# JJanai/slowflow

Measured on AMD Instinct MI355X. Metric: Mpix*solver-iters/s at 1024x436 (whole coarse-to-fine path), higher is better.
Workload: dtype f32

## Files before the change

slowflow_amd/csrc/job.hip:

```cpp
#include <algorithm>
#include <cmath>
#include <cstring>
#include <memory>
#include <vector>

#include "sfa_internal.h"

#pragma clang fp contract(off)

namespace sfa {

enum { P_WX = 0, P_WY, P_UU, P_VV, P_DU, P_DV, P_ODU, P_ODV, P_SH, P_SV, P_A11, P_A12, P_A22, P_B1, P_B2, P_OCC, P_DPSIS, P_COUNT };
struct Level {
    int w = 0, h = 0, pitch = 0, lstride = 0, ref = 0, F = 0, nb = 0;
    bool fused = true;
    long pl = 0, es = 0;
    long off_masks = 0, off_warp = 0, off_stacks = 0, off_tmp = 0;
    float *base = nullptr;
    float *pbase = nullptr;
    float *plane(int i) const { return i < 2 ? pbase + (long)i * pl : base + (long)(i - 2) * pl; }
    float *mask(int s) const { return base + off_masks + (long)s * pl; }
    float *stack(int s, int toref) const { return base + off_stacks + ((long)s * 2 + toref) * 24 * pl; }
    float *warp(int s, int sp1) const { return base + off_warp + (long)(s + sp1) * 3 * pl; }
    float *frame(int f) const { return pbase + 2 * pl + (long)f * 3 * pl; }
    float *tmp() const { return base + off_tmp; }
    Geo geo() const { return Geo{w, h, pitch, pl, es, nb, WMask::first(nb), nullptr}; }
    Geo geo(const WMask &active) const { return Geo{w, h, pitch, pl, es, nb, active, nullptr}; }
    static long persistent_floats(int pitch, int h, int ref) { return (long)pitch * h * (2 + (2L * ref + 1) * 3); }
    static long transient_floats(int pitch, int h, int ref, bool fused) {
        return (long)pitch * h * ((P_COUNT - 2) + 2 * ref + (2L * ref + 1) * 3 + (fused ? 0 : 2L * ref * 2 * 24));
    }
    void layout(float *transient, float *persistent, int w_, int h_, int lstride_, int ref_, int nb_, long es_, bool fused_) {
        base = transient; pbase = persistent; w = w_; h = h_; pitch = dev_pitch(w_); lstride = lstride_; ref = ref_; F = 2 * ref_ + 1; nb = nb_; es = es_; fused = fused_;
        pl = (long)pitch * h;
        off_masks = (long)(P_COUNT - 2) * pl;
        off_warp = off_masks + 2L * ref * pl;
        off_stacks = off_warp + (2L * ref + 1) * 3 * pl;
        off_tmp = off_warp;
    }
};
struct ChannelWeights { const float *dev = nullptr; long pl = 0, es = 0; int pitch = 0, stride0 = 0; };

static const float *pair_image(const Level &L, int s, int sp1) { return (s + sp1 - L.ref == 0) ? L.frame(s + sp1) : L.warp(s, sp1); }

static bool get_derivatives(sfa_ctx *c, const Level &L, const sfa_params &p, const Geo &g, const bool need_toref[2 * SFA_MAX_REF], bool with_smoothness = false) {
    const int ref = L.ref;
    WarpJobs J;
    J.n = 0;
    for (int f = p.one_direction ? ref + 1 : 0; f <= 2 * ref; f++) {
        if (f == ref) continue;
        const int s = f < ref ? f : f - 1;
        J.job[J.n++] = WarpJob{L.frame(f) - L.base, L.warp(f < ref ? f : f - 1, f < ref ? 0 : 1) - L.base, L.mask(s) - L.base, f - ref};
    }
    const bool smoothed = with_smoothness && L.fused &&
                          launch_warp_smooth(c, g, J, L.base, L.plane(P_WX), L.plane(P_WY), p.smoothing, L.plane(P_SH), L.plane(P_SV), L.plane(P_DPSIS), p.alpha, pen(p.robust_reg));
    if (!smoothed) launch_warp_jobs(c, g, J, L.base, L.plane(P_WX), L.plane(P_WY));
    for (int s = p.one_direction ? ref : 0; s < 2 * ref; s++) {
        if (L.fused) continue;
        const float *w_s = pair_image(L, s, 0), *w_sp1 = pair_image(L, s, 1);
        launch_deriv_stack(c, g, L.stack(s, 0), w_s, w_sp1, L.es, L.es);
        if (need_toref[s]) {
            if (s < ref) launch_deriv_stack(c, g, L.stack(s, 1), w_s, L.frame(ref), L.es, L.es);
            else         launch_deriv_stack(c, g, L.stack(s, 1), L.frame(ref), w_sp1, L.es, L.es);
        }
    }
    return smoothed;
}

static int optimize_occlusions(sfa_ctx *c, const Level &L, const sfa_params &p, const Geo &g, DevMem &scratch) {
    const int ref = L.ref;
    const size_t n = (size_t)L.nb * L.pl;
    SFA_TRY(scratch.alloc(c, (2 + kCutWorkPlanes) * n * sizeof(float)));
    float *d0 = scratch.f(), *d1 = d0 + n, *work = d1 + n;
    OccArgs oa;
    memset(&oa, 0, sizeof oa);
    oa.nslots = 2 * ref; oa.hd = p.delta / 3.0f; oa.hg = p.gamma / 3.0f; oa.penalty = p.occlusion_penalty;
    oa.color = pen(p.robust_color); oa.grad = pen(p.robust_grad);
    for (int s = 0; s < 2 * ref; s++) {
        const float *i1 = pair_image(L, s, 0), *i2 = pair_image(L, s, 1);
        const float *r1 = s < ref ? i1 : L.frame(ref), *r2 = s < ref ? L.frame(ref) : i2;
        const int idx = std::max(ref - s - 1, s - ref);
        oa.slot[s] = OccSlot{i1 - L.base, i2 - L.base, r1 - L.base, r2 - L.base, L.off_masks + (long)s * L.pl, p.rho[idx], p.omega[idx], s >= ref ? 0 : 1};
    }
    launch_occ_costs(c, g, oa, L.base, d0, d1, L.pl);
    return run_grid_cut(c, g, L.plane(P_OCC), L.es, d0, d1, work, p.occlusion_alpha);
}


static Term data_term(const Level &L, const sfa_params &p, int slot, int is_ref, float weight, float s) {
    const float *i1 = pair_image(L, slot, 0), *i2 = pair_image(L, slot, 1);
    if (is_ref) { if (slot < L.ref) i2 = L.frame(L.ref); else i1 = L.frame(L.ref); }
    return Term{L.off_stacks + ((long)slot * 2 + is_ref) * 24 * L.pl, L.off_masks + (long)slot * L.pl, weight * (p.delta / 3.0f), weight * (p.gamma / 3.0f), s, is_ref,
                i1 - L.base, i2 - L.base, slot < L.ref};
}
static int data_terms(sfa_ctx *c, const Level &L, const sfa_params &p, const ChannelWeights &cw, AssembleArgs &aa, bool need_toref[2 * SFA_MAX_REF]) {
    const int ref = L.ref;
    memset(&aa, 0, sizeof aa);
    for (int s = 0; s < ref; s++) {
        const int a = ref - 1 - s;
        if (!p.one_direction) {
            if (p.rho[a] > 0) aa.t[aa.n++] = data_term(L, p, s, 0, p.rho[a], (float)(s - ref));
            if (p.omega[a] > 0) { aa.t[aa.n++] = data_term(L, p, s, 1, p.omega[a], (float)(s - ref)); need_toref[s] = true; }
        }
        if (p.rho[s] > 0) aa.t[aa.n++] = data_term(L, p, ref + s, 0, p.rho[s], (float)s);
        if (p.omega[s] > 0) { aa.t[aa.n++] = data_term(L, p, ref + s, 1, p.omega[s], (float)(s + 1)); need_toref[ref + s] = true; }
        aa.data_norm += p.rho[s] + p.omega[s];
    }
    for (int t = 0; t < aa.n; t++)
        if (aa.t[t].is_ref && aa.t[t].s == 0) return set_error(c, SFA_ERR_REF_FRAME, "Frame compared to reference frame is the reference frame itself!");
    aa.one_direction = p.one_direction; aa.dt_norm = p.dataterm_norm;
    aa.color = pen(p.robust_color); aa.grad = pen(p.robust_grad);
    aa.chw = cw.dev; aa.chw_pl = cw.pl; aa.chw_es = cw.es; aa.chw_pitch = cw.pitch; aa.chw_stride0 = cw.stride0; aa.lstride = L.lstride;
    aa.accumulate = 0; aa.do_laplacian = 1;
    return SFA_OK;
}

struct LevelPlan {
    bool verbose;
    bool red_black;
    bool direct;
    bool uv_alias;
    bool thres_in, thres_out;
    float *wx, *wy, *uu, *vv, *du, *dv, *odu, *odv, *sh, *sv, *a11, *a12, *a22, *b1, *b2, *occ, *dpsis, *UU, *VV;
    float *dfa, *dfb, *ifa, *ifb;
    LevelPlan(const sfa_ctx *c, const Level &L, const sfa_params &p) {
        verbose = c->verbose_changes;
        red_black = p.sor_order == 1;
        direct = L.fused && !red_black && !sw_given(Switches::NO_DIRECT_OPERANDS);
        uv_alias = direct && p.niter_inner == 1 && !sw_given(Switches::NO_UV_ALIAS) && !verbose;
        thres_in = p.thres_inner > 0; thres_out = p.thres_outer > 0;
        wx = L.plane(P_WX); wy = L.plane(P_WY); uu = L.plane(P_UU); vv = L.plane(P_VV); du = L.plane(P_DU); dv = L.plane(P_DV);
        odu = L.plane(P_ODU); odv = L.plane(P_ODV); sh = L.plane(P_SH); sv = L.plane(P_SV); a11 = L.plane(P_A11); a12 = L.plane(P_A12);
        a22 = L.plane(P_A22); b1 = L.plane(P_B1); b2 = L.plane(P_B2); occ = L.plane(P_OCC); dpsis = L.plane(P_DPSIS);
        UU = uv_alias ? wx : uu; VV = uv_alias ? wy : vv;
        dfa = thres_out && !sw_given(Switches::NO_EXACT_BREAK) ? a11 : nullptr; dfb = dfa ? a12 : nullptr;
        ifa = thres_in && !sw_given(Switches::NO_EXACT_BREAK) ? a11 : nullptr; ifb = ifa ? a12 : nullptr;
    }
};

struct OuterBreak {
    sfa_ctx *c; bool on;
    int known(int n, WMask &active) const {
        if (!on || n < kMaskLag) return SFA_OK;
        const int slot = (n - kMaskLag) % kMaskRing;
        SFA_HIP(c, hipEventSynchronize(c->ev_mask[slot]));
        for (int i = 0; i < kMaskWords; i++) active.w[i] = *(volatile unsigned long long *)&c->h_amask[slot].w[i];
        return SFA_OK;
    }
    int publish(int n) const {
        if (!on) return SFA_OK;
        const int slot = n % kMaskRing;
        SFA_HIP(c, hipMemcpyAsync(&c->h_amask[slot], c->d_amask, sizeof(WMask), hipMemcpyDeviceToHost, c->stream));
        SFA_HIP(c, hipEventRecord(c->ev_mask[slot], c->stream));
        return SFA_OK;
    }
};

static void print_changes(sfa_ctx *c, const Level &L, const char *what, int it, const WMask &who) {
    if (hipMemcpyAsync(c->h_red, c->d_red, 2 * L.nb * sizeof(double), hipMemcpyDeviceToHost, c->stream) != hipSuccess || hipStreamSynchronize(c->stream) != hipSuccess) return;
    const double n = (double)L.w * L.h;
    for (int b = 0; b < L.nb; b++)
        if (who.test(b)) {
            if (L.nb > 1) printf("[window %d] ", b);
            printf("%s %d\tavg change %g,%g\n", what, it, (double)(float)(c->h_red[2 * b] / n), (double)(float)(c->h_red[2 * b + 1] / n));
        }
    fflush(stdout);
}

static int assemble_and_solve(sfa_ctx *c, const Level &L, const sfa_params &p, const LevelPlan &P, AssembleArgs &aa, SorWorkspace &sorws, const Geo &gi, bool first_zero,
                       bool smoothed) {
    if (!first_zero) launch_copy_planes(c, gi, P.odu, P.du, 2, L.es, L.es);
    if (!smoothed) launch_smoothness(c, gi, p.smoothing, P.sh, P.sv, P.UU, P.VV, P.dpsis, p.alpha, pen(p.robust_reg));
    aa.op = SorOperandOut();
    aa.zero_duv = first_zero ? 1 : 0;
    if (P.direct) SFA_TRY(sor_operand_target(c, sorws, gi, p.niter_solver, &aa.op));
    if (L.fused) SFA_TRY(launch_assemble_images(c, gi, aa, L.base, P.a11, P.a12, P.a22, P.b1, P.b2, P.du, P.dv, P.UU, P.VV, P.sh, P.sv, P.occ));
    else launch_assemble(c, gi, aa, L.base, P.a11, P.a12, P.a22, P.b1, P.b2, P.du, P.dv, P.uu, P.vv, P.sh, P.sv);
    if (P.direct) return sor_run_prepared(c, sorws, gi, nullptr, nullptr, p.niter_solver, p.sor_omega);
    if (P.red_black) return sor_rb_run(c, gi, P.du, P.dv, P.a11, P.a12, P.a22, P.b1, P.b2, P.sh, P.sv, p.niter_solver, p.sor_omega);
    return sor_run(c, sorws, gi, P.du, P.dv, P.a11, P.a12, P.a22, P.b1, P.b2, P.sh, P.sv, p.niter_solver, p.sor_omega, false);
}

static bool update_flow(sfa_ctx *c, const sfa_params &p, const LevelPlan &P, const SorOperandOut &x, const Geo &gi, int inner, bool first_zero) {
    const bool last = inner + 1 == p.niter_inner;
    float *const ia = last ? nullptr : P.ifa, *const ib = last ? nullptr : P.ifb;
    if (P.direct && last && !P.verbose) {
        launch_update_outer_x(c, gi, P.uv_alias ? nullptr : P.uu, P.uv_alias ? nullptr : P.vv, P.wx, P.wy, x, c->d_red, P.dfa, P.dfb);
        return true;
    }
    if (P.direct)
        launch_update_inner_x(c, gi, P.uu, P.vv, P.wx, P.wy, x, first_zero ? nullptr : P.odu, first_zero ? nullptr : P.odv, last ? nullptr : P.du,
                              last ? nullptr : P.dv, c->d_red, ia, ib);
    else
        launch_update_inner(c, gi, P.uu, P.vv, P.wx, P.wy, P.du, P.dv, P.odu, P.odv, c->d_red, ia, ib);
    return false;
}

static int inner_break(sfa_ctx *c, const Level &L, const sfa_params &p, const LevelPlan &P, const Geo &gi, WMask &in_active) {
    const double npx = (double)L.h * L.w;
    SFA_HIP(c, hipMemcpyAsync(c->h_red, c->d_red, 2 * L.nb * sizeof(double), hipMemcpyDeviceToHost, c->stream));
    SFA_HIP(c, hipStreamSynchronize(c->stream));
    WMask close = WMask::none();
    for (int b = 0; b < L.nb; b++)
        if (in_active.test(b)) {
            const double ad = c->h_red[2 * b] / npx, dd = c->h_red[2 * b + 1] / npx, dm = (ad < dd) ? dd : ad;
            if (P.ifa && fabs(dm - (double)p.thres_inner) <= break_band(L.w, L.h) * (double)p.thres_inner) { close.set(b); continue; }
            if (std::max((float)ad, (float)dd) < p.thres_inner) in_active.clear(b);
        }
    if (!close.any()) return SFA_OK;
    float *const dx = c->d_last->exact;
    const float *const hx = reinterpret_cast<const LastBlock *>(c->h_red)->exact;
    launch_exact_norms(c, gi, P.ifa, P.ifb, close, dx);
    SFA_HIP(c, hipMemcpyAsync(const_cast<float *>(hx), dx, 2 * L.nb * sizeof(float), hipMemcpyDeviceToHost, c->stream));
    SFA_HIP(c, hipStreamSynchronize(c->stream));
    for (int b = 0; b < L.nb; b++)
        if (close.test(b) && std::max(hx[2 * b], hx[2 * b + 1]) < p.thres_inner) in_active.clear(b);
    return SFA_OK;
}

static int inner_iterations(sfa_ctx *c, const Level &L, const sfa_params &p, const LevelPlan &P, AssembleArgs &aa, SorWorkspace &sorws, const Geo &g, bool smoothed) {
    if (!P.direct) launch_zero_planes(c, g, P.du, 2);
    WMask in_active = g.active, outer_done = WMask::none();
    for (int inner = 0; inner < p.niter_inner; inner++) {
        Geo gi = g;
        gi.active = in_active;
        const bool first_zero = P.direct && inner == 0;
        SFA_TRY(assemble_and_solve(c, L, p, P, aa, sorws, gi, first_zero, smoothed && inner == 0));
        if (update_flow(c, p, P, aa.op, gi, inner, first_zero)) outer_done = in_active;
        if (P.verbose) print_changes(c, L, "\tinner it", inner, in_active);
// ... 457 lines not shown
```

slowflow_amd/csrc/kernels.hip:

```cpp
#include "sfa_device.h"
#include "sor_device.h"

#pragma clang fp contract(off)

namespace sfa {

__device__ __forceinline__ float psi_vec(const PenaltyDev &p, float xsq) {
    const float e2 = p.eps * p.eps;
    switch (p.id) {
    case 0: return 1.0f;
    case 2: return __fdiv_rn(1.0f, 2.0f * e2 + xsq);
    case 3: {
        float out = __fdiv_rn(1.0f, 2.0f * sqrt_rn(xsq + e2));
        if (sqrt_rn(xsq) > p.trunc) out = 0.0f;
        return out;
    }
    case 4: {
        float t = e2 + xsq;
        t = t * t;
        return __fdiv_rn(e2 + 2.0f * xsq, t);
    }
    default: return __fdiv_rn(1.0f, 2.0f * sqrt_rn(xsq + e2));
    }
}
__device__ __forceinline__ float psi_scalar(const PenaltyDev &p, float xsq) {
    const float e2f = p.eps * p.eps;
    const double e2d = (double)e2f;
    switch (p.id) {
    case 0: return 1.0f;
    case 2: return (float)(1.0 / (2.0 * e2d + (double)xsq));
    case 3:
        if (sqrt_rn(xsq) > p.trunc) return 0.0f;
        return __fdiv_rn(1.0f, 2.0f * sqrt_rn(xsq + e2f));
    case 4: {
        float t = (float)(e2d + (double)xsq);
        t = t * t;
        return (float)((e2d + (double)(2.0f * xsq)) / (double)t);
    }
    default: return (float)(1.0 / (2.0 * __dsqrt_rn((double)xsq + e2d)));
    }
}

__global__ void k_warp(float *__restrict__ dst3, float *__restrict__ mask, const float *__restrict__ src3, const float *__restrict__ wx,
                       const float *__restrict__ wy, Geo g, int factor, long src_es) {
    const int b = blockIdx.z;
    if (!elem_active(g, b)) return;
    const int x = blockIdx.x * BX + threadIdx.x, y = blockIdx.y * BY + threadIdx.y;
    if (x >= g.w || y >= g.h) return;
    dst3 += b * g.es; wx += b * g.es; wy += b * g.es; src3 += b * src_es;
    const size_t o = (size_t)y * g.pitch + x;
    if (factor == 0) {
        for (int k = 0; k < 3; k++) dst3[k * g.pl + o] = src3[k * g.pl + o];
        return;
    }
    const float xx = x + factor * wx[o];
    const float yy = y + factor * wy[o];
    const int xi = floor_to_int_x86(xx), yi = floor_to_int_x86(yy);
    const float dx = xx - xi, dy = yy - yi;
    if (mask) mask[b * g.es + o] = (xx >= 0 && xx <= g.w - 1 && yy >= 0 && yy <= g.h - 1) ? 1.0f : 0.0f;
    const int x1 = clampi(xi, 0, g.w - 1), x2 = clampi(xi + 1, 0, g.w - 1);
    const int y1 = clampi(yi, 0, g.h - 1), y2 = clampi(yi + 1, 0, g.h - 1);
    const float ax = 1.0f - dx, ay = 1.0f - dy;
    for (int k = 0; k < 3; k++) {
        const float *s = src3 + k * g.pl;
        dst3[k * g.pl + o] = s[(size_t)y1 * g.pitch + x1] * ax * ay + s[(size_t)y1 * g.pitch + x2] * dx * ay
                           + s[(size_t)y2 * g.pitch + x1] * ax * dy + s[(size_t)y2 * g.pitch + x2] * dx * dy;
    }
}
template <bool ALLJ>
__global__ void k_warp_jobs(WarpJobs J, float *__restrict__ base, const float *__restrict__ wx, const float *__restrict__ wy, Geo g) {
    const int b = ALLJ ? blockIdx.z : blockIdx.z / J.n, j0 = ALLJ ? 0 : blockIdx.z % J.n;
    if (!elem_active(g, b)) return;
    const int x = blockIdx.x * BX + threadIdx.x, y = blockIdx.y * BY + threadIdx.y;
    if (x >= g.w || y >= g.h) return;
    const long eb = b * g.es;
    const size_t o = (size_t)y * g.pitch + x;
    const float fx0 = wx[eb + o], fy0 = wy[eb + o];
    for (int j = j0; j <= (ALLJ ? J.n - 1 : j0); j++) {
        const int factor = J.job[j].factor;
        const float *src3 = base + eb + J.job[j].src_off;
        float *dst3 = base + eb + J.job[j].dst_off;
        const float xx = x + factor * fx0;
        const float yy = y + factor * fy0;
        const int xi = floor_to_int_x86(xx), yi = floor_to_int_x86(yy);
        const float dx = xx - xi, dy = yy - yi;
        if (J.job[j].mask_off >= 0) base[eb + J.job[j].mask_off + o] = (xx >= 0 && xx <= g.w - 1 && yy >= 0 && yy <= g.h - 1) ? 1.0f : 0.0f;
        const int x1 = clampi(xi, 0, g.w - 1), x2 = clampi(xi + 1, 0, g.w - 1);
        const int y1 = clampi(yi, 0, g.h - 1), y2 = clampi(yi + 1, 0, g.h - 1);
        const float ax = 1.0f - dx, ay = 1.0f - dy;
        float out[3];
#pragma unroll
        for (int k = 0; k < 3; k++) {
            const float *s = src3 + k * g.pl;
            out[k] = s[(size_t)y1 * g.pitch + x1] * ax * ay + s[(size_t)y1 * g.pitch + x2] * dx * ay
                   + s[(size_t)y2 * g.pitch + x1] * ax * dy + s[(size_t)y2 * g.pitch + x2] * dx * dy;
// ... 1226 lines not shown
        for (int ch = 0; ch < 3; ch++) {
            const TileAcc X{sX[ch], x0, y0 + 2}, Y{sY[ch], x0, y0 + 2}, Z{sZ[ch], x0, y0};
            p.ixy[ch] = d5y(X, xc_, y, g.h);
            p.iyy[ch] = d5y(Y, xc_, y, g.h);
            p.iyz[ch] = d5y(Z, xc_, y, g.h);
            p.ix[ch] = sX[ch][c]; p.iy[ch] = sY[ch][c]; p.iz[ch] = sZ[ch][cz];
            p.ixx[ch] = d5x_in(sX[ch], c);
            p.ixz[ch] = d5x_in(sZ[ch], cz);
        }
    }
    return p;
}
template <class K>
__device__ __forceinline__ void asm_epilogue_pixel(const AssembleArgs &a, const Geo &g, Acc &A, float u, float v, int x0, int y0, int tx, int yl, int x, int y) {
    const float *const lds = asm_lds<K>();
    const int gy0 = y0 + DT_H - 1;
    const TileAcc U{lds, x0, gy0}, V{lds + K::GR * DT_W, x0, gy0}, Hh{lds + 2 * K::GR * DT_W, x0, gy0}, Wv{lds + 3 * K::GR * DT_W, x0, gy0};
    if (a.do_laplacian) {
        A.b1 = laplacian_gather(A.b1, U, Hh, Wv, x, y, g.w, g.h);
        A.b2 = laplacian_gather(A.b2, V, Hh, Wv, x, y, g.w, g.h);
    }
    if (!a.op.sa) return;
    const float hp = Hh(x, y);
    const float hl = x > 0 ? Hh(x - 1, y) : 0.0f;
    const float vp = Wv(x, y);
    const float vt = y > 0 ? Wv(x, y - 1) : 0.0f;
    const PointBlock q = sor_point_block(hl, hp, vt, vp, y, g.h, A.a11, A.a12, A.a22);
    const OperandTile<K> T;
    T.A[yl][tx] = make_float4(q.i11, q.i12, q.i22, vt);
    T.B[yl][tx] = make_float4(A.b1, A.b2, hp, y < g.h - 1 ? vp : 0.0f);
    T.X[yl][tx] = make_float2(u, v);
}
template <class K>
__device__ __forceinline__ void asm_store_operand_tile(const SorOperandOut &op, const Geo &g, int b, int c0, int r0) {
    const OperandTile<K> T;
    for (int item = threadIdx.x; item < (DT_X + K::TY - 1) * K::TY; item += K::NT) {
        const int dl = item / K::TY, rl = item % K::TY, cl = dl - rl;
        if (cl < 0 || cl >= DT_X) continue;
        const int r = r0 + rl, c = c0 + cl;
        if (r >= g.h || c >= g.w) continue;
        const size_t e = diag_entry(b, op.ent, op.RP, op.G, c, r);
        if (SFA_X_AI & 64) continue;
        const float2 xv = T.X[rl][cl];
        op.sa[e] = T.A[rl][cl];
        op.sb[e] = T.B[rl][cl];
        op.x[e] = f2u(xv.x, xv.y);
    }
}

template <int TY, int NT, int MINB, bool ZUV, int FAST, bool XT>
__global__ void __launch_bounds__(NT, MINB) k_assemble_images(AssembleArgs a, const float *__restrict__ base, float *__restrict__ a11, float *__restrict__ a12,
                                                              float *__restrict__ a22, float *__restrict__ b1, float *__restrict__ b2,
                                                              const float *__restrict__ du, const float *__restrict__ dv, const float *__restrict__ uu,
                                                              const float *__restrict__ vv, const float *__restrict__ sh, const float *__restrict__ sv,
                                                              const float *__restrict__ occ, Geo g, XcdTiles xt) {
    using K = AsmTile<TY, NT>;
    constexpr int NR = K::NR, NP = K::NP;
    float *const lds = asm_lds<K>();
#ifdef SFA_ASM_TIMING
    unsigned long long at_acc[14] = {0}, at_t = __builtin_readcyclecounter();
#endif
    int bx, by, b;
    if (!asm_block_tile<XT>(g, xt, bx, by, b)) return;
    asm_reset_progress<K>(a.op, bx, by, b);
    if (!elem_active(g, b)) return;
    const int x0 = bx * DT_X - DT_H, y0 = by * TY - DT_H;
    const bool tile_in = SFA_TILE_FAST && x0 >= 0 && x0 + DT_W <= g.w && y0 >= 0 && y0 + K::TR <= g.h;
    const long eb = b * g.es;
    const int tx = threadIdx.x & 63;
    const int ty = __builtin_amdgcn_readfirstlane(threadIdx.x >> 6);
    const int x = x0 + DT_H + tx;
    const int dt_norm = FAST ? 1 : a.dt_norm;
    PenaltyDev pcolor = a.color, pgrad = a.grad;
    if (FAST) { pcolor.id = FAST; pgrad.id = FAST; }
    Acc A[NP];
    float u[NP], v[NP], wk[NP][3], fwd[NP], bwd[NP], oc[NP];
    bool ok[NP];
#pragma unroll
    for (int k = 0; k < NP; k++) {
        const int y = y0 + DT_H + ty + NR * k;
        ok[k] = x < g.w && y < g.h;
        A[k].a11 = A[k].a12 = A[k].a22 = A[k].b1 = A[k].b2 = 0.0f;
        u[k] = v[k] = 0.0f; fwd[k] = bwd[k] = 0.0f; oc[k] = 0.0f;
        wk[k][0] = wk[k][1] = wk[k][2] = 1.0f;
        if (!ok[k]) continue;
        const size_t o = (size_t)y * g.pitch + x;
        if (!ZUV) { u[k] = du[eb + o]; v[k] = dv[eb + o]; }
        if (!FAST && a.chw) channel_weights(a, b, x, y, wk[k]);
        if (!(SFA_X_AI & 128)) oc[k] = occ[eb + o];
    }
    const bool need_g = a.do_laplacian || a.op.sa;
    auto stage_epilogue_operands = [&]() {
        if (!need_g) return;
        for (int i0 = 0; i0 < K::NGQ; i0 += NT) {
            const int item = i0 + (int)threadIdx.x;
            const int q = item % K::QM, row = (item / K::QM) % K::GR, pl = item / (K::QM * K::GR);
            const int gy = y0 + DT_H - 1 + row, gx = x0 + 4 * q;
            const float *src = pl == 0 ? uu : pl == 1 ? vv : pl == 2 ? sh : sv;
            if (!(SFA_X_AI & 32) && item < K::NGQ && gy >= 0 && gy < g.h && gx >= 0 && gx + 3 < g.pitch && (pl >= 2 || a.do_laplacian))
                dma16(src + eb + (size_t)gy * g.pitch + gx, lds_addr(lds + 4 * (i0 + 64 * ty)));
        }
    };
    AT_MARK(13);
    if (a.n == 0) stage_epilogue_operands();
    float mk[NP];
    for (int t = 0; t < a.n; t++) {
        const Term &T = a.t[t];
        AT_MARK(0);
        if (t > 0) __syncthreads();
        AT_MARK(1);
        SFA_PRIO(SFA_PRIO_STAGE);
        asm_issue_image_dma<K>(base + eb + T.i1_off, base + eb + T.i2_off, g, x0, y0, tx, ty);
#pragma unroll
        for (int k = 0; k < NP; k++) {
            const size_t o = (size_t)(y0 + DT_H + ty + NR * k) * g.pitch + x;
            mk[k] = ok[k] && !(SFA_X_AI & 128) ? base[eb + T.mask_off + o] : 0.0f;
        }
        AT_MARK(2);
        asm volatile("s_waitcnt vmcnt(0)" ::: "memory");
#pragma unroll
        for (int k = 0; k < NP; k++) {
            asm volatile("" : "+v"(mk[k]), "+v"(oc[k]));
            if (!FAST) asm volatile("" : "+v"(wk[k][0]), "+v"(wk[k][1]), "+v"(wk[k][2]));
            if (!ZUV) asm volatile("" : "+v"(u[k]), "+v"(v[k]));
        }
        AT_MARK(3);
        __syncthreads();
        AT_MARK(4);
        if (t == 0) {
#pragma unroll
            for (int k = 0; k < NP; k++) mask_weights(oc[k], a.data_norm, fwd[k], bwd[k]);
        }
        if (tile_in) asm_convert<K, true>(base + eb + T.i1_off, base + eb + T.i2_off, g, x0, y0);
        else asm_convert<K, false>(base + eb + T.i1_off, base + eb + T.i2_off, g, x0, y0);
        AT_MARK(5);
        AT_MARK(0);
        __syncthreads();
        AT_MARK(6);
        SFA_PRIO(SFA_PRIO_STAGE);
        if (tile_in) asm_stage1<K, true>(g, x0, y0);
        else asm_stage1<K, false>(g, x0, y0);
        AT_MARK(7);
        __syncthreads();
        AT_MARK(8);
        SFA_PRIO(0);
        if (t == a.n - 1) stage_epilogue_operands();
#pragma unroll
        for (int k = 0; k < NP; k++) {
            const int yl = ty + NR * k, y = y0 + DT_H + yl;
            if (y >= g.h) break;
            Px p = asm_pixel_derivatives<K>(g, x0, y0, tx, yl, y);
#pragma unroll
            for (int ch = 0; ch < 3; ch++) p.wk[ch] = FAST ? 1.0f : wk[k][ch];
            if (!ok[k]) continue;
            float m = mk[k];
            if (!a.one_direction || !T.backward) m = T.backward ? 1.0f * bwd[k] * m : 1.0f * fwd[k] * m;
            if (SFA_X_AI & 16) {
                for (int ch = 0; ch < 3; ch++) {
                    A[k].a11 += p.ix[ch] + p.ixx[ch] + m; A[k].a12 += p.iy[ch] + p.ixy[ch]; A[k].a22 += p.iz[ch] + p.iyy[ch]; A[k].b1 += p.ixz[ch]; A[k].b2 += p.iyz[ch];
                }
            } else if (T.is_ref) term_ref<ZUV, FAST != 0>(A[k], p, m, u[k], v[k], T.hd, T.hg, T.s, dt_norm, pcolor, pgrad, a.chain_ok != 0);
            else          term_succ<ZUV, FAST != 0>(A[k], p, m, u[k], v[k], T.hd, T.hg, T.s, dt_norm, pcolor, pgrad, a.chain_ok != 0);
        }
    }
    AT_MARK(0);
    if (need_g) {
        asm volatile("s_waitcnt vmcnt(0)" ::: "memory");
        __syncthreads();
    }
    AT_MARK(9);
    SFA_PRIO(SFA_PRIO_STAGE);
#pragma unroll
    for (int k = 0; k < NP; k++) {
        if (!ok[k]) continue;
        const int yl = ty + NR * k, y = y0 + DT_H + yl;
        asm_epilogue_pixel<K>(a, g, A[k], u[k], v[k], x0, y0, tx, yl, x, y);
        if (!a.op.sa) {
            const size_t o = eb + (size_t)y * g.pitch + x;
            a11[o] = A[k].a11; a12[o] = A[k].a12; a22[o] = A[k].a22; b1[o] = A[k].b1; b2[o] = A[k].b2;
        }
    }
    if (!a.op.sa) return;
    AT_MARK(10);
    __syncthreads();
    AT_MARK(11);
    asm_store_operand_tile<K>(a.op, g, b, x0 + DT_H, y0 + DT_H);
#ifdef SFA_ASM_TIMING
    AT_MARK(12);
    if ((threadIdx.x & 63) == 0 && (bx + 3 * by + 7 * b) % 61 == 0)
        for (int i = 0; i < 14; i++) atomicAdd(&g_asm_timing[i], at_acc[i]);
#endif
}
using AsmKernel = decltype(&k_assemble_images<kAsmTY, kAsmNT, kAsmMinWaves, true, 1, true>);
template <bool ZUV, int FAST>
static AsmKernel asm_kernel(bool xcd) {
    return xcd ? k_assemble_images<kAsmTY, kAsmNT, kAsmMinWaves, ZUV, FAST, true> : k_assemble_images<kAsmTY, kAsmNT, kAsmMinWaves, ZUV, FAST, false>;
}
int launch_assemble_images(sfa_ctx *c, const Geo &g, const AssembleArgs &a_in, const float *base, float *a11, float *a12, float *a22, float *b1, float *b2,
                           const float *du, const float *dv, const float *uu, const float *vv, const float *sh, const float *sv, const float *occ) {
    AssembleArgs a = a_in;
    if ((unsigned long long)g.pl * 12ull >= (1ull << 32)) return set_error(c, SFA_ERR_ARG, "k_assemble_images: plane of %ld entries is beyond the kernel's 32-bit offsets", g.pl);
    const bool prof = c->profile && c->ev2_used + 2 <= c->ev2.size();
    if (prof) (void)hipEventRecord(c->ev2[c->ev2_used], c->stream);
    auto is_modl1 = [](int id) { return id != 0 && id != 2 && id != 3 && id != 4; };
    const bool foldable = a.dt_norm == 1 && !a.chw && !sw_given(Switches::ASSEMBLE_GENERIC);
    const int fast = !foldable ? 0 : (is_modl1(a.color.id) && is_modl1(a.grad.id)) ? 1 : (a.color.id == 2 && a.grad.id == 2) ? 2 : 0;
    {
        auto in = [](float v, float lo, float hi) { return v >= lo && v <= hi; };
        const float elo = fast == 2 ? 1.0f / 1024 : 1.0f / 1048576, ehi = fast == 2 ? 1024.0f : 1048576.0f, hlo = fast == 2 ? 1.0f / 4096 : 1.0f / 65536;
        bool okp = fast != 0 && in(a.data_norm, 1.0f / 256, 256.0f) && in(a.color.eps, elo, ehi) && in(a.grad.eps, elo, ehi);
        for (int t = 0; t < a.n && okp; t++) okp = (a.t[t].hd == 0.0f || in(a.t[t].hd, hlo, 65536.0f)) && (a.t[t].hg == 0.0f || in(a.t[t].hg, hlo, 65536.0f));
        a.chain_ok = okp && !sw_given(Switches::EXACT_DIV) ? 1 : 0;
    }
    const dim3 grid_((g.w + DT_X - 1) / DT_X, (g.h + kAsmTY - 1) / kAsmTY, g.nb);
    const bool xcd_env = sw_int(Switches::ASM_XCD, 1) != 0;
    const long ntiles = (long)grid_.x * grid_.y * grid_.z;
    const bool xcd = xcd_env && ntiles >= 64 && ntiles < (1l << 30);
    const XcdTiles xt{(int)grid_.x, (int)grid_.y, (int)((ntiles + 7) / 8)};
    const dim3 grid1_(8u * (unsigned)xt.chunk, 1, 1);
    const AsmKernel kern = a.zero_duv ? (fast == 1 ? asm_kernel<true, 1>(xcd) : fast == 2 ? asm_kernel<true, 2>(xcd) : asm_kernel<true, 0>(xcd))
                                      : (fast == 1 ? asm_kernel<false, 1>(xcd) : fast == 2 ? asm_kernel<false, 2>(xcd) : asm_kernel<false, 0>(xcd));
    hipLaunchKernelGGL(kern, xcd ? grid1_ : grid_, dim3(kAsmNT), 0, c->stream, a, base, a11, a12, a22, b1, b2, du, dv, uu, vv, sh, sv, occ, g, xt);
    if (prof) {
        (void)hipEventRecord(c->ev2[c->ev2_used + 1], c->stream);
        c->ev2_used += 2;
        c->asm_pixel_terms += (double)g.w * g.h * g.nb * a.n;
    }
    return SFA_OK;
}

__device__ __forceinline__ double wave_sum(double v) {
#pragma unroll
    for (int off = 32; off > 0; off >>= 1) v += __shfl_down(v, off, 64);
    return v;
}
__device__ __forceinline__ void block_sum2(double &a, double &b) {
    __shared__ double sm[2 * BY];
    a = wave_sum(a);
    b = wave_sum(b);
    const int wid = threadIdx.y, lane = threadIdx.x;
    if (lane == 0) { sm[wid] = a; sm[BY + wid] = b; }
    __syncthreads();
    if (wid == 0 && lane == 0) {
        double sa = 0, sb = 0;
        for (int i = 0; i < BY; i++) { sa += sm[i]; sb += sm[BY + i]; }
        a = sa; b = sb;
    }
}

__global__ void __launch_bounds__(BX *BY) k_update_inner(float *__restrict__ uu, float *__restrict__ vv, const float *__restrict__ wx, const float *__restrict__ wy,
                                                          const float *__restrict__ du, const float *__restrict__ dv, const float *__restrict__ odu,
                                                          const float *__restrict__ odv, double *__restrict__ partial, float *__restrict__ dfa, float *__restrict__ dfb, Geo g) {
    const int b = blockIdx.z;
    const int x = blockIdx.x * BX + threadIdx.x;
    double sa = 0, sb = 0;
    if (elem_active(g, b) && x < g.w)
        for (int y = blockIdx.y * BY + threadIdx.y; y < g.h; y += gridDim.y * BY) {
            const size_t o = b * g.es + (size_t)y * g.pitch + x;
            const float d = du[o], e = dv[o];
            sa += (double)fabsf(odu[o] - d);
            sb += (double)fabsf(odv[o] - e);
            if (dfa) { dfa[o] = fabsf(odu[o] - d); dfb[o] = fabsf(odv[o] - e); }
            uu[o] = wx[o] + d;
            vv[o] = wy[o] + e;
        }
    block_sum2(sa, sb);
    if (threadIdx.x == 0 && threadIdx.y == 0) {
        const size_t blk = ((size_t)b * gridDim.y + blockIdx.y) * gridDim.x + blockIdx.x;
        partial[2 * blk] = sa; partial[2 * blk + 1] = sb;
    }
}
__global__ void __launch_bounds__(BX *BY) k_update_inner_x(float *__restrict__ uu, float *__restrict__ vv, const float *__restrict__ wx, const float *__restrict__ wy,
                                                            const unsigned long long *__restrict__ xs, long ent, int RP, int G, const float *__restrict__ odu,
                                                            const float *__restrict__ odv, float *__restrict__ du_out, float *__restrict__ dv_out,
                                                            double *__restrict__ partial, float *__restrict__ dfa, float *__restrict__ dfb, Geo g) {
// ... 680 lines not shown
```

slowflow_amd/csrc/sfa_internal.h:

```cpp
#pragma once
#include <hip/hip_runtime.h>

#include <cstdarg>
#include <cstdio>
#include <string>
#include <vector>

#include "../../include/slowflow_amd.h"
#include "dev_view.h"

#pragma clang fp contract(off)

namespace sfa {

constexpr int kMaskWords = 2;
constexpr int kMaxBatch = 64 * kMaskWords;
struct WMask {
    unsigned long long w[kMaskWords];
    __host__ __device__ bool test(int b) const { return (w[b >> 6] >> (b & 63)) & 1ull; }
    __host__ __device__ void clear(int b) { w[b >> 6] &= ~(1ull << (b & 63)); }
    __host__ __device__ void set(int b) { w[b >> 6] |= 1ull << (b & 63); }
    __host__ __device__ bool any() const { unsigned long long o = 0; for (int i = 0; i < kMaskWords; i++) o |= w[i]; return o != 0; }
    __host__ __device__ bool operator==(const WMask &o) const { bool e = true; for (int i = 0; i < kMaskWords; i++) e = e && w[i] == o.w[i]; return e; }
    __host__ __device__ bool operator!=(const WMask &o) const { return !(*this == o); }
// ... 144 lines not shown
    double acc_jc, acc_cv, acc_bc, acc_gc, acc_occ, acc_temporal_occ;
    float thr, fb_thr;
    int penalty;
    double eps_sq;
    float weight;
};
struct EnergyPlan { AdaptTab tab; EnergyArgs a; int rJ, J, w, h, gw, gh, incr, start, r, NN; size_t lds; };
int energy_plan(sfa_ctx *ctx, const sfa_energy_params *p, int r_Jets, int Jets, int w, int h, EnergyPlan *out);
void energy_records_device(sfa_ctx *ctx, size_t nf, int w, int h, const float *frames, float *der, void *rec);
struct EnergyWork { double *U, *V; unsigned long long *occ; float *jc, *oc; double *ep; };
int energies_device(sfa_ctx *ctx, const EnergyPlan &pl, int n, const double *acc_u, const double *acc_v, const int *tracked, const void *rec, bool identity,
                    const void *fwd, const void *bwd, const EnergyWork &wk, double *energy, unsigned long long *occ_out, size_t out_seg, double *adapted_u,
                    double *adapted_v, size_t adapted_seg);
int energies_adapted_device(sfa_ctx *ctx, const EnergyPlan &pl, int n, const int *tracked, const EnergyWork &wk, double *adapted_u, double *adapted_v, size_t adapted_seg);
struct FuseWork {
    const double *U, *V, *energy; const unsigned long long *occ; const float *weight;
    unsigned char *nl, *lab; double *theta, *P, *M; unsigned char *xcur, *xbest;
    int *slot; double *fu, *fv; unsigned char *out_occ; double *seg_energy, *seg_bound; int *seg_iters;
};
int fuse_device(sfa_ctx *ctx, const sfa_fuse_params *p, int n, int K, int Jets, int w, int h, int gw, int gh, const FuseWork &f, hipEvent_t *ev);

struct Geo { int w, h, pitch; long pl; long es; int nb; WMask active; const unsigned long long *amask; };

struct PenaltyDev { int id; float eps, trunc; };
inline PenaltyDev pen(const sfa_penalty &p) { return PenaltyDev{p.id, p.eps, p.trunc}; }

struct WarpJob { long src_off, dst_off, mask_off; int factor; };
struct WarpJobs { WarpJob job[4 * SFA_MAX_REF]; int n; };
void launch_warp_jobs(sfa_ctx *c, const Geo &g, const WarpJobs &J, float *base, const float *wx, const float *wy);
bool launch_warp_smooth(sfa_ctx *c, const Geo &g, const WarpJobs &J, float *base, const float *wx, const float *wy, int method, float *sh, float *sv,
                        const float *dpsis, float alpha, PenaltyDev reg);
void launch_warp(sfa_ctx *c, const Geo &g, float *dst3, float *mask, const float *src3, const float *wx, const float *wy, int factor,
                 long src_es );
void launch_deriv_stack(sfa_ctx *c, const Geo &g, float *out24, const float *I1, const float *I2, long es1, long es2);
void launch_convolve(sfa_ctx *c, const Geo &g, float *dst, const float *src, int order, int horiz, int nplanes);
void launch_dpsis(sfa_ctx *c, const Geo &g, float *dst, const float *im3, long im_es, float coef, const float avg[3], const float stdv[3], int hbit);
void launch_smoothness(sfa_ctx *c, const Geo &g, int method, float *sh, float *sv, const float *uu, const float *vv, const float *dpsis,
                       float alpha, PenaltyDev reg);
void launch_sub_laplacian(sfa_ctx *c, const Geo &g, float *dst, const float *src, const float *wh, const float *wv);
void launch_mask_weight(sfa_ctx *c, const Geo &g, float *masks, const float *occ, float data_norm, int ref, int one_direction);
void launch_fill(sfa_ctx *c, float *p, size_t n, float v);
void launch_division_chain(sfa_ctx *c, const float *a, const float *b, float *q_chain, float *q_exact, unsigned char *admitted, size_t n);
void launch_fill_planes(sfa_ctx *c, const Geo &g, float *p, int nplanes, float v);
void launch_zero_planes(sfa_ctx *c, const Geo &g, float *p, int nplanes);
void launch_outer_threshold(sfa_ctx *c, const Geo &g, const double *red, float thres, const float *dfa = nullptr, const float *dfb = nullptr);
void launch_set_mask(sfa_ctx *c, const WMask &v);

struct SorOperandOut {
    float4 *sa = nullptr, *sb = nullptr; unsigned long long *x = nullptr; unsigned *flags = nullptr;
    long ent = 0; int RP = 0, G = 0, ntasks = 0, nb = 0;
};
struct Term {
    long stack_off; long mask_off; float hd, hg, s; int is_ref;
    long i1_off, i2_off; int backward;
};
struct AssembleArgs {
    Term t[kMaxTerms];
    int n;
    int dt_norm;
    PenaltyDev color, grad;
    const float *chw; long chw_pl; long chw_es; int chw_pitch; int chw_stride0; int lstride;
    int accumulate;
    int do_laplacian;
    float data_norm; int one_direction;
    SorOperandOut op;
    int zero_duv;
    int chain_ok = 0;
};
void launch_assemble(sfa_ctx *c, const Geo &g, const AssembleArgs &a, const float *base , float *a11, float *a12,
                     float *a22, float *b1, float *b2, const float *du, const float *dv, const float *uu, const float *vv, const float *sh, const float *sv);

int launch_assemble_images(sfa_ctx *c, const Geo &g, const AssembleArgs &a, const float *base, float *a11, float *a12, float *a22, float *b1, float *b2,
                            const float *du, const float *dv, const float *uu, const float *vv, const float *sh, const float *sv, const float *occ);

void launch_smoothness_2f(sfa_ctx *c, const Geo &g, float *sh, float *sv, const float *uu, const float *vv, const float *dpsis, float half_alpha);
void launch_data_2f(sfa_ctx *c, const Geo &g, const float *D, const float *mask, const float *du, const float *dv, float *a11, float *a12, float *a22, float *b1,
                    float *b2, const float *wx, const float *wy, const float *sh, const float *sv, float hd, float hg);
void launch_data_2f_fused(sfa_ctx *c, const Geo &g, const float *I1, const float *I2, const float *mask, const float *du, const float *dv, float *a11, float *a12,
                          float *a22, float *b1, float *b2, const float *wx, const float *wy, const float *sh, const float *sv, float hd, float hg);

struct OccSlot {
    long s1_off, s2_off;
    long r1_off, r2_off;
    long mask_off;
    float rho, omega;
    int label;
};
struct OccArgs { OccSlot slot[2 * SFA_MAX_REF]; int nslots; float hd, hg, penalty; PenaltyDev color, grad; };
void launch_occ_costs(sfa_ctx *c, const Geo &g, const OccArgs &a, const float *base, float *d0, float *d1, long d_es );
constexpr int kCutWorkPlanes = 13;
int run_grid_cut(sfa_ctx *c, const Geo &g, float *occ, long occ_es, const float *d0, const float *d1, float *work, float alpha);

void launch_update_inner(sfa_ctx *c, const Geo &g, float *uu, float *vv, const float *wx, const float *wy, const float *du, const float *dv,
                         const float *old_du, const float *old_dv, double *red , float *dfa = nullptr, float *dfb = nullptr);
void launch_update_inner_x(sfa_ctx *c, const Geo &g, float *uu, float *vv, const float *wx, const float *wy, const SorOperandOut &x, const float *old_du,
                           const float *old_dv, float *du_out, float *dv_out, double *red, float *dfa = nullptr, float *dfb = nullptr);
void launch_exact_norms(sfa_ctx *c, const Geo &g, const float *dfa, const float *dfb, const WMask &which, float *out);
void launch_update_outer_x(sfa_ctx *c, const Geo &g, float *uu, float *vv, float *wx, float *wy, const SorOperandOut &x, double *red, float *dfa = nullptr,
                           float *dfb = nullptr);
void launch_update_outer(sfa_ctx *c, const Geo &g, float *wx, float *wy, const float *uu, const float *vv, double *red, float *dfa = nullptr, float *dfb = nullptr);
void launch_copy_planes(sfa_ctx *c, const Geo &g, float *dst, const float *src, int nplanes, long dst_es, long src_es);
void launch_scale_plane(sfa_ctx *c, const Geo &g, float *p, float s);

void launch_gauss_blur(sfa_ctx *c, const Geo &g, float *dst, float *tmp, const float *src, int nplanes, const float *taps, int radius);
void launch_resize(sfa_ctx *c, float *dst, int dw, int dh, int dpitch, long dpl, long des, const float *src, int sw, int sh, int spitch, long spl, long ses,
                   int nplanes, int nb, float post_scale);
void launch_resize_flow(sfa_ctx *c, float *dstx, float *dsty, int dw, int dh, int dpitch, long des, const float *srcx, const float *srcy, int sw, int sh, int spitch,
                        long ses, int nb, float post_x, float post_y);
void launch_resize_scaled(sfa_ctx *c, float *dst, int dw, int dh, int dpitch, long dpl, long des, const float *src, int sw, int sh, int spitch, long spl,
                          long ses, int nplanes, int nb, float post_scale, double scale_x, double scale_y);
bool launch_pyr_down(sfa_ctx *c, float *dst, int dw, int dh, int dpitch, long dpl, long des, const float *src, int sw, int sh, int spitch, long spl, long ses,
                     int nplanes, int nb, const float *taps, int radius);
void launch_presmooth(sfa_ctx *c, const Geo &g, float *dst, float *tmp, const float *src, int nplanes, float sigma);
void launch_normalize_sums(sfa_ctx *c, const Geo &g, const float *frames3, double *red );
void launch_normalize_apply(sfa_ctx *c, const Geo &g, float *frames3, const double avg[3], const double stdv[3]);
__attribute__((visibility("hidden"))) int cv_gauss_taps(float sigma, float *k);

struct PackSrc { const void *p; int dtype; long long sw, sf, sc, sr, sx; };
void launch_pack_frames(sfa_ctx *c, float *dst, long dst_es, long pl, int pitch, int w, int h, int nwin, int F, const PackSrc &s);
void launch_pack_flow(sfa_ctx *c, float *dst, long dst_es, long pl, int pitch, int w, int h, int nwin, const float *src, const long long st[4]);
void launch_unpack_planes(sfa_ctx *c, const float *wx, const float *wy, const float *occ, long src_es, int pitch, int w, int h, int nwin, float *flow,
                          const long long st[4], float *occ_dst, const long long ost[3]);

struct MosaicSrc { const void *p; int dtype; long long sf, sr, sx; int W, H, x0, y0; };
struct MosaicDst { float *p; long long sf, sc, sr, sx; int w, h; };
void launch_demosaic(sfa_ctx *c, const MosaicSrc &src, const MosaicDst &dst, int n, int method, int red_x, int red_y);
// ... 61 lines not shown
```

Baseline: 256,100.

## Recompute warp validity masks in assemble kernel instead of storing and reloading them

The fused assemble kernel now derives each term's out-of-bounds warp mask from the flow planes wx/wy and a per-term mask factor, packed into a bitfield, instead of loading a stored mask plane per term. The warp kernels skip writing mask planes when they are not needed elsewhere (fused path without two-direction occlusion reasoning). Mask-weight setup is also moved out of the term loop and done once after the first image stage. This removes per-term mask loads and mask-plane writes at the cost of two extra flow loads and a little ALU per pixel, and it depends on the warp kernel handling a -1 mask offset, which is not shown.

```diff
diff --git a/slowflow_amd/csrc/job.hip b/slowflow_amd/csrc/job.hip
--- a/slowflow_amd/csrc/job.hip
+++ b/slowflow_amd/csrc/job.hip
@@ -42,15 +42,17 @@
 struct ChannelWeights { const float *dev = nullptr; long pl = 0, es = 0; int pitch = 0, stride0 = 0; };
 
 static const float *pair_image(const Level &L, int s, int sp1) { return (s + sp1 - L.ref == 0) ? L.frame(s + sp1) : L.warp(s, sp1); }
+static int mask_factor(const Level &L, int s) { return (s < L.ref ? s : s + 1) - L.ref; }
 
 static bool get_derivatives(sfa_ctx *c, const Level &L, const sfa_params &p, const Geo &g, const bool need_toref[2 * SFA_MAX_REF], bool with_smoothness = false) {
     const int ref = L.ref;
     WarpJobs J;
     J.n = 0;
+    const bool store_masks = !L.fused || (p.occlusion_reasoning && !p.one_direction);
     for (int f = p.one_direction ? ref + 1 : 0; f <= 2 * ref; f++) {
         if (f == ref) continue;
         const int s = f < ref ? f : f - 1;
-        J.job[J.n++] = WarpJob{L.frame(f) - L.base, L.warp(f < ref ? f : f - 1, f < ref ? 0 : 1) - L.base, L.mask(s) - L.base, f - ref};
+        J.job[J.n++] = WarpJob{L.frame(f) - L.base, L.warp(f < ref ? f : f - 1, f < ref ? 0 : 1) - L.base, store_masks ? L.mask(s) - L.base : -1L, mask_factor(L, s)};
     }
     const bool smoothed = with_smoothness && L.fused &&
                           launch_warp_smooth(c, g, J, L.base, L.plane(P_WX), L.plane(P_WY), p.smoothing, L.plane(P_SH), L.plane(P_SV), L.plane(P_DPSIS), p.alpha, pen(p.robust_reg));
@@ -91,7 +93,7 @@
     const float *i1 = pair_image(L, slot, 0), *i2 = pair_image(L, slot, 1);
     if (is_ref) { if (slot < L.ref) i2 = L.frame(L.ref); else i1 = L.frame(L.ref); }
     return Term{L.off_stacks + ((long)slot * 2 + is_ref) * 24 * L.pl, L.off_masks + (long)slot * L.pl, weight * (p.delta / 3.0f), weight * (p.gamma / 3.0f), s, is_ref,
-                i1 - L.base, i2 - L.base, slot < L.ref};
+                i1 - L.base, i2 - L.base, slot < L.ref, mask_factor(L, slot)};
 }
 static int data_terms(sfa_ctx *c, const Level &L, const sfa_params &p, const ChannelWeights &cw, AssembleArgs &aa, bool need_toref[2 * SFA_MAX_REF]) {
     const int ref = L.ref;
@@ -174,7 +176,7 @@
     aa.op = SorOperandOut();
     aa.zero_duv = first_zero ? 1 : 0;
     if (P.direct) SFA_TRY(sor_operand_target(c, sorws, gi, p.niter_solver, &aa.op));
-    if (L.fused) SFA_TRY(launch_assemble_images(c, gi, aa, L.base, P.a11, P.a12, P.a22, P.b1, P.b2, P.du, P.dv, P.UU, P.VV, P.sh, P.sv, P.occ));
+    if (L.fused) SFA_TRY(launch_assemble_images(c, gi, aa, L.base, P.a11, P.a12, P.a22, P.b1, P.b2, P.du, P.dv, P.UU, P.VV, P.wx, P.wy, P.sh, P.sv, P.occ));
     else launch_assemble(c, gi, aa, L.base, P.a11, P.a12, P.a22, P.b1, P.b2, P.du, P.dv, P.uu, P.vv, P.sh, P.sv);
     if (P.direct) return sor_run_prepared(c, sorws, gi, nullptr, nullptr, p.niter_solver, p.sor_omega);
     if (P.red_black) return sor_rb_run(c, gi, P.du, P.dv, P.a11, P.a12, P.a22, P.b1, P.b2, P.sh, P.sv, p.niter_solver, p.sor_omega);
diff --git a/slowflow_amd/csrc/kernels.hip b/slowflow_amd/csrc/kernels.hip
--- a/slowflow_amd/csrc/kernels.hip
+++ b/slowflow_amd/csrc/kernels.hip
@@ -41,6 +41,11 @@
     }
 }
 
+__device__ __forceinline__ bool warp_mask(int x, int y, int factor, float fx, float fy, int w, int h) {
+    const float xx = x + factor * fx;
+    const float yy = y + factor * fy;
+    return xx >= 0 && xx <= w - 1 && yy >= 0 && yy <= h - 1;
+}
 __global__ void k_warp(float *__restrict__ dst3, float *__restrict__ mask, const float *__restrict__ src3, const float *__restrict__ wx,
                        const float *__restrict__ wy, Geo g, int factor, long src_es) {
     const int b = blockIdx.z;
@@ -1373,8 +1378,9 @@
 __global__ void __launch_bounds__(NT, MINB) k_assemble_images(AssembleArgs a, const float *__restrict__ base, float *__restrict__ a11, float *__restrict__ a12,
                                                               float *__restrict__ a22, float *__restrict__ b1, float *__restrict__ b2,
                                                               const float *__restrict__ du, const float *__restrict__ dv, const float *__restrict__ uu,
-                                                              const float *__restrict__ vv, const float *__restrict__ sh, const float *__restrict__ sv,
-                                                              const float *__restrict__ occ, Geo g, XcdTiles xt) {
+                                                              const float *__restrict__ vv, const float *__restrict__ wx, const float *__restrict__ wy,
+                                                              const float *__restrict__ sh, const float *__restrict__ sv, const float *__restrict__ occ, Geo g,
+                                                              XcdTiles xt) {
     using K = AsmTile<TY, NT>;
     constexpr int NR = K::NR, NP = K::NP;
     float *const lds = asm_lds<K>();
@@ -1395,20 +1401,21 @@
     PenaltyDev pcolor = a.color, pgrad = a.grad;
     if (FAST) { pcolor.id = FAST; pgrad.id = FAST; }
     Acc A[NP];
-    float u[NP], v[NP], wk[NP][3], fwd[NP], bwd[NP], oc[NP];
+    float u[NP], v[NP], wk[NP][3], fwd[NP], bwd[NP], oc[NP], fx[NP], fy[NP];
+    unsigned mb[NP];
     bool ok[NP];
 #pragma unroll
     for (int k = 0; k < NP; k++) {
         const int y = y0 + DT_H + ty + NR * k;
         ok[k] = x < g.w && y < g.h;
         A[k].a11 = A[k].a12 = A[k].a22 = A[k].b1 = A[k].b2 = 0.0f;
-        u[k] = v[k] = 0.0f; fwd[k] = bwd[k] = 0.0f; oc[k] = 0.0f;
+        u[k] = v[k] = 0.0f; fwd[k] = bwd[k] = 0.0f; oc[k] = 0.0f; fx[k] = fy[k] = 0.0f; mb[k] = 0u;
         wk[k][0] = wk[k][1] = wk[k][2] = 1.0f;
         if (!ok[k]) continue;
         const size_t o = (size_t)y * g.pitch + x;
         if (!ZUV) { u[k] = du[eb + o]; v[k] = dv[eb + o]; }
         if (!FAST && a.chw) channel_weights(a, b, x, y, wk[k]);
-        if (!(SFA_X_AI & 128)) oc[k] = occ[eb + o];
+        if (!(SFA_X_AI & 128)) { oc[k] = occ[eb + o]; fx[k] = wx[eb + o]; fy[k] = wy[eb + o]; }
     }
     const bool need_g = a.do_laplacian || a.op.sa;
     auto stage_epilogue_operands = [&]() {
@@ -1424,34 +1431,39 @@
     };
     AT_MARK(13);
     if (a.n == 0) stage_epilogue_operands();
-    float mk[NP];
+    auto stage_term_images = [&](const Term &T) {
+        SFA_PRIO(SFA_PRIO_STAGE);
+        asm_issue_image_dma<K>(base + eb + T.i1_off, base + eb + T.i2_off, g, x0, y0, tx, ty);
+        AT_MARK(2);
+        asm volatile("s_waitcnt vmcnt(0)" ::: "memory");
+        AT_MARK(3);
+    };
+    if (a.n > 0) {
+        AT_MARK(1);
+        stage_term_images(a.t[0]);
+#pragma unroll
+        for (int k = 0; k < NP; k++) {
+            asm volatile("" : "+v"(oc[k]), "+v"(fx[k]), "+v"(fy[k]));
+            if (!FAST) asm volatile("" : "+v"(wk[k][0]), "+v"(wk[k][1]), "+v"(wk[k][2]));
+            if (!ZUV) asm volatile("" : "+v"(u[k]), "+v"(v[k]));
+            mask_weights(oc[k], a.data_norm, fwd[k], bwd[k]);
+            unsigned bits = 0u;
+            for (int tt = 0; tt < a.n; tt++)
+                bits |= (warp_mask(x, y0 + DT_H + ty + NR * k, a.t[tt].mask_factor, fx[k], fy[k], g.w, g.h) ? 1u : 0u) << tt;
+            mb[k] = ok[k] && !(SFA_X_AI & 128) ? bits : 0u;
+        }
+        AT_MARK(5);
+    }
     for (int t = 0; t < a.n; t++) {
         const Term &T = a.t[t];
         AT_MARK(0);
-        if (t > 0) __syncthreads();
-        AT_MARK(1);
-        SFA_PRIO(SFA_PRIO_STAGE);
-        asm_issue_image_dma<K>(base + eb + T.i1_off, base + eb + T.i2_off, g, x0, y0, tx, ty);
-#pragma unroll
-        for (int k = 0; k < NP; k++) {
-            const size_t o = (size_t)(y0 + DT_H + ty + NR * k) * g.pitch + x;
-            mk[k] = ok[k] && !(SFA_X_AI & 128) ? base[eb + T.mask_off + o] : 0.0f;
-        }
-        AT_MARK(2);
-        asm volatile("s_waitcnt vmcnt(0)" ::: "memory");
-#pragma unroll
-        for (int k = 0; k < NP; k++) {
-            asm volatile("" : "+v"(mk[k]), "+v"(oc[k]));
-            if (!FAST) asm volatile("" : "+v"(wk[k][0]), "+v"(wk[k][1]), "+v"(wk[k][2]));
-            if (!ZUV) asm volatile("" : "+v"(u[k]), "+v"(v[k]));
-        }
-        AT_MARK(3);
+        if (t > 0) {
+            __syncthreads();
+            AT_MARK(1);
+            stage_term_images(T);
+        }
         __syncthreads();
         AT_MARK(4);
-        if (t == 0) {
-#pragma unroll
-            for (int k = 0; k < NP; k++) mask_weights(oc[k], a.data_norm, fwd[k], bwd[k]);
-        }
         if (tile_in) asm_convert<K, true>(base + eb + T.i1_off, base + eb + T.i2_off, g, x0, y0);
         else asm_convert<K, false>(base + eb + T.i1_off, base + eb + T.i2_off, g, x0, y0);
         AT_MARK(5);
@@ -1474,7 +1486,7 @@
 #pragma unroll
             for (int ch = 0; ch < 3; ch++) p.wk[ch] = FAST ? 1.0f : wk[k][ch];
             if (!ok[k]) continue;
-            float m = mk[k];
+            float m = ((mb[k] >> t) & 1u) ? 1.0f : 0.0f;
             if (!a.one_direction || !T.backward) m = T.backward ? 1.0f * bwd[k] * m : 1.0f * fwd[k] * m;
             if (SFA_X_AI & 16) {
                 for (int ch = 0; ch < 3; ch++) {
@@ -1518,7 +1530,8 @@
     return xcd ? k_assemble_images<kAsmTY, kAsmNT, kAsmMinWaves, ZUV, FAST, true> : k_assemble_images<kAsmTY, kAsmNT, kAsmMinWaves, ZUV, FAST, false>;
 }
 int launch_assemble_images(sfa_ctx *c, const Geo &g, const AssembleArgs &a_in, const float *base, float *a11, float *a12, float *a22, float *b1, float *b2,
-                           const float *du, const float *dv, const float *uu, const float *vv, const float *sh, const float *sv, const float *occ) {
+                           const float *du, const float *dv, const float *uu, const float *vv, const float *wx, const float *wy, const float *sh, const float *sv,
+                           const float *occ) {
     AssembleArgs a = a_in;
     if ((unsigned long long)g.pl * 12ull >= (1ull << 32)) return set_error(c, SFA_ERR_ARG, "k_assemble_images: plane of %ld entries is beyond the kernel's 32-bit offsets", g.pl);
     const bool prof = c->profile && c->ev2_used + 2 <= c->ev2.size();
@@ -1541,7 +1554,7 @@
     const dim3 grid1_(8u * (unsigned)xt.chunk, 1, 1);
     const AsmKernel kern = a.zero_duv ? (fast == 1 ? asm_kernel<true, 1>(xcd) : fast == 2 ? asm_kernel<true, 2>(xcd) : asm_kernel<true, 0>(xcd))
                                       : (fast == 1 ? asm_kernel<false, 1>(xcd) : fast == 2 ? asm_kernel<false, 2>(xcd) : asm_kernel<false, 0>(xcd));
-    hipLaunchKernelGGL(kern, xcd ? grid1_ : grid_, dim3(kAsmNT), 0, c->stream, a, base, a11, a12, a22, b1, b2, du, dv, uu, vv, sh, sv, occ, g, xt);
+    hipLaunchKernelGGL(kern, xcd ? grid1_ : grid_, dim3(kAsmNT), 0, c->stream, a, base, a11, a12, a22, b1, b2, du, dv, uu, vv, wx, wy, sh, sv, occ, g, xt);
     if (prof) {
         (void)hipEventRecord(c->ev2[c->ev2_used + 1], c->stream);
         c->ev2_used += 2;
diff --git a/slowflow_amd/csrc/sfa_internal.h b/slowflow_amd/csrc/sfa_internal.h
--- a/slowflow_amd/csrc/sfa_internal.h
+++ b/slowflow_amd/csrc/sfa_internal.h
@@ -220,8 +220,9 @@
 };
 struct Term {
     long stack_off; long mask_off; float hd, hg, s; int is_ref;
-    long i1_off, i2_off; int backward;
-};
+    long i1_off, i2_off; int backward; int mask_factor;
+};
+static_assert(kMaxTerms <= 32, "k_assemble_images keeps one mask bit per term in a 32-bit word");
 struct AssembleArgs {
     Term t[kMaxTerms];
     int n;
@@ -239,7 +240,8 @@
                      float *a22, float *b1, float *b2, const float *du, const float *dv, const float *uu, const float *vv, const float *sh, const float *sv);
 
 int launch_assemble_images(sfa_ctx *c, const Geo &g, const AssembleArgs &a, const float *base, float *a11, float *a12, float *a22, float *b1, float *b2,
-                            const float *du, const float *dv, const float *uu, const float *vv, const float *sh, const float *sv, const float *occ);
+                            const float *du, const float *dv, const float *uu, const float *vv, const float *wx, const float *wy, const float *sh, const float *sv,
+                            const float *occ);
 
 void launch_smoothness_2f(sfa_ctx *c, const Geo &g, float *sh, float *sv, const float *uu, const float *vv, const float *dpsis, float half_alpha);
 void launch_data_2f(sfa_ctx *c, const Geo &g, const float *D, const float *mask, const float *du, const float *dv, float *a11, float *a12, float *a22, float *b1,
```

Result: no change. 258,200, median of 6 (+0.8%).
